# TritonDataCenter/containerpilot

Measured on AMD Instinct MI355X. Metric: events/sec, higher is better.
Workload: dtype n/a (CPU daemon, no tensor math; see BASELINE.json north_star); 1 GPU; model=containerpilot daemon, BASELINE stress shape scaled to 550 jobs, jobs=550, watches=50, parallelism=1 independent daemons (1/rank)

## Files before the change

### cpp/include/cpilot/loop.hpp

```cpp
#pragma once

#include <sys/types.h>

#include <chrono>
#include <cstdint>
#include <deque>
#include <functional>
#include <map>
#include <memory>
#include <mutex>
#include <queue>
#include <vector>

namespace cpilot {

using Clock = std::chrono::steady_clock;
using TimePoint = Clock::time_point;
using Ns = std::chrono::nanoseconds;

std::function<void()> timedItem(const char* tag, std::function<void()> fn);
void dumpItemTags();

void resetThreadScheduling();

class Loop {
 public:
  using FdCallback = std::function<void(uint32_t epollEvents)>;
  using TimerCallback = std::function<void()>;
  using ChildCallback = std::function<void(int waitStatus)>;

  Loop();
  ~Loop();

  Loop(const Loop&) = delete;
  Loop& operator=(const Loop&) = delete;

  void watchFd(int fd, uint32_t events, FdCallback cb);
  void modifyFd(int fd, uint32_t events);
  void unwatchFd(int fd);

  uint64_t addTimeout(Ns delay, TimerCallback cb);
  uint64_t addInterval(Ns interval, TimerCallback cb, Ns initialDelay = Ns(-1));
  void cancelTimer(uint64_t id);

  void defer(std::function<void()> fn);

  void post(std::function<void()> fn);

  void watchChild(pid_t pid, ChildCallback cb);
  void reapChildren();
  void notifyChildExit(pid_t pid, int status);

  static void postIfLive(Loop* loop, uint64_t id, std::function<void()> fn);
  uint64_t id() const { return id_; }

  void run();
  void stop();

  bool stopped() const { return stopped_; }

 private:
  struct Timer {
    uint64_t id;
    TimePoint deadline;
    Ns interval;
    TimerCallback cb;
    bool canceled = false;
  };
  struct TimerCmp {
    bool operator()(const std::shared_ptr<Timer>& a,
                    const std::shared_ptr<Timer>& b) const {
      return a->deadline > b->deadline;
    }
  };

  void armTimerFd();
  void fireDueTimers();
  void drainDeferred();
  void drainPosted();

  uint64_t id_ = 0;
  int epfd_ = -1;
  int timerfd_ = -1;
  int wakeupFds_[2] = {-1, -1};
  bool stopped_ = false;

  std::map<int, FdCallback> fdCallbacks_;
  std::priority_queue<std::shared_ptr<Timer>,
                      std::vector<std::shared_ptr<Timer>>, TimerCmp>
      timers_;
  std::map<uint64_t, std::shared_ptr<Timer>> timersById_;
  uint64_t nextTimerId_ = 1;

  std::deque<std::function<void()>> deferred_;

  std::mutex postedMu_;
  std::deque<std::function<void()>> posted_;

  std::map<pid_t, ChildCallback> children_;
  std::map<pid_t, int> unclaimedExits_;
};

}
```

### cpp/include/cpilot/spawner.hpp

```cpp
#pragma once

#include <sys/types.h>

#include <cstdint>
#include <deque>
#include <functional>
#include <map>
#include <memory>
#include <mutex>
#include <string>
#include <thread>
#include <vector>

#include "cpilot/loop.hpp"

namespace cpilot {

class Spawner {
 public:
  using SpawnCb = std::function<void(pid_t pid, int err)>;

  static Spawner& global();

  void spawn(Loop& loop, const std::string& execPath,
             const std::vector<std::string>& args,
             std::shared_ptr<const std::vector<std::string>> baseEnv,
             const std::vector<std::string>& extraEnv, int stdioFd,
             SpawnCb cb);

  int helperCount() const { return (int)helpers_.size(); }

  size_t backlog();
  bool overloaded();

 private:
  Spawner();
  struct Helper {
    int sock = -1;
    pid_t pid = -1;
    bool dead = false;
    std::deque<std::pair<std::vector<char>, int>> overflow;
    std::mutex sendMu;
  };
  struct Pending {
    Loop* loop;
    uint64_t loopId;
    SpawnCb cb;
    size_t helperIdx;
  };

  bool launchHelper(Helper* h);
  void flushOverflow(size_t idx);
  void readerMain();
  void handleMessage(size_t idx, const char* buf, size_t len);
  void helperDied(size_t idx);
  bool sendRequest(Helper& h, const std::vector<char>& buf, int fd);
  void wakeReader();

  std::string helperPath_;
  std::vector<std::unique_ptr<Helper>> helpers_;
  size_t nextHelper_ = 0;

  std::mutex mu_;
  std::map<uint32_t, Pending> pending_;
  uint32_t nextReqId_ = 1;
  std::map<pid_t, std::pair<Loop*, uint64_t>> pidLoops_;

  int wakeFds_[2] = {-1, -1};
  std::thread reader_;
};

}
```

### cpp/include/cpilot/spawnproto.hpp

```cpp
#pragma once

#include <cstdint>

namespace cpilot {
namespace spawnproto {

constexpr int kHelperFd = 3;

enum MsgType : uint32_t {
  kSpawnRequest = 1,
  kSpawnReply = 2,
  kChildExit = 3,
};

struct RequestHeader {
  uint32_t type;
  uint32_t reqId;
  uint32_t argc;
  uint32_t envc;
  uint8_t wantStdio;
  uint8_t pad[3];
};

struct Reply {
  uint32_t type;
  uint32_t reqId;
  int32_t pid;
  int32_t err;
};

struct ExitNotice {
  uint32_t type;
  uint32_t pad;
  int32_t pid;
  int32_t status;
};

constexpr size_t kMaxRequestBytes = 1024 * 1024;

}
}
```

### cpp/src/command.cpp

```cpp
#include "cpilot/command.hpp"

#include <fcntl.h>
#include <signal.h>
#include <sys/epoll.h>
#include <sys/wait.h>
#include <unistd.h>

#include <cctype>
#include <cstring>
#include <cstdio>
#include <map>

#include "cpilot/log.hpp"
#include "cpilot/spawner.hpp"

extern char** environ;

namespace cpilot {

namespace {

std::map<std::string, std::string>& pidEnvOverlay() {
  static std::map<std::string, std::string> overlay;
  return overlay;
}

std::shared_ptr<const std::vector<std::string>>& baseEnvCache() {
  static std::shared_ptr<const std::vector<std::string>> cache;
  return cache;
}
bool& baseEnvDirty() {
  static bool dirty = true;
  return dirty;
}

std::shared_ptr<const std::vector<std::string>> baseEnvSnapshot() {
  if (!baseEnvDirty() && baseEnvCache()) return baseEnvCache();
  auto& overlay = pidEnvOverlay();
  auto env = std::make_shared<std::vector<std::string>>();
  for (char** e = ::environ; *e; e++) {
    const char* eq = strchr(*e, '=');
    if (eq && overlay.count(std::string(*e, eq - *e))) continue;
    env->emplace_back(*e);
  }
  baseEnvCache() = env;
  baseEnvDirty() = false;
  return baseEnvCache();
}

std::vector<std::string>& overlayStrings() {
  static std::vector<std::string> strings;
  return strings;
}
std::map<std::string, size_t>& overlayIndex() {
  static std::map<std::string, size_t> index;
  return index;
}

const std::vector<std::string>& overlayExtras() { return overlayStrings(); }

void overlaySet(const std::string& key, const std::string& value) {
  auto [it, inserted] = pidEnvOverlay().emplace(key, value);
  if (inserted) {
    overlayIndex()[key] = overlayStrings().size();
    overlayStrings().push_back(key + "=" + value);
    if (getenv(key.c_str())) baseEnvDirty() = true;
  } else {
    it->second = value;
    overlayStrings()[overlayIndex()[key]] = key + "=" + value;
  }
}

void overlayErase(const std::string& key) {
  if (pidEnvOverlay().erase(key)) {
    auto idxIt = overlayIndex().find(key);
    if (idxIt != overlayIndex().end()) {
      size_t slot = idxIt->second;
      overlayIndex().erase(idxIt);
      auto& strs = overlayStrings();
      if (slot + 1 != strs.size()) {
        strs[slot] = std::move(strs.back());
        size_t eq = strs[slot].find('=');
        overlayIndex()[strs[slot].substr(0, eq)] = slot;
      }
      strs.pop_back();
    }
    if (getenv(key.c_str())) baseEnvDirty() = true;
  }
}

}

void commandEnvInvalidate() { baseEnvDirty() = true; }

bool parseArgs(const Json& raw, std::string* execPath,
               std::vector<std::string>* args, std::string* err) {
  std::vector<std::string> all;
  if (raw.isString()) {
    std::string s = raw.str();
    size_t a = 0, b = s.size();
    while (a < b && isspace((unsigned char)s[a])) a++;
    while (b > a && isspace((unsigned char)s[b - 1])) b--;
    s = s.substr(a, b - a);
    if (!s.empty()) {
      std::string cur;
      for (char c : s) {
        if (c == ' ') {
          all.push_back(cur);
          cur.clear();
        } else {
          cur += c;
        }
      }
      all.push_back(cur);
    }
  } else if (raw.isArray()) {
    for (auto& e : raw.array()) {
      if (e.isString()) all.push_back(e.str());
      else all.push_back(e.dump());
    }
  } else if (!raw.isNull()) {
    *err = "unable to parse exec arguments";
    return false;
  }
  if (all.empty()) {
    *err = "received zero-length argument";
    return false;
  }
  *execPath = all[0];
  args->assign(all.begin() + 1, all.end());
  return true;
}

CommandPtr newCommand(const Json& rawExec, Duration timeout, bool raw,
                      const std::string& logField, std::string* err) {
  std::string execPath;
  std::vector<std::string> args;
  if (!parseArgs(rawExec, &execPath, &args, err)) return nullptr;
  return std::make_shared<Command>(execPath, args, timeout, raw, logField);
}

Command::Command(std::string execPath, std::vector<std::string> args,
                 Duration timeout, bool raw, std::string logField)
    : name_(execPath),
      exec_(std::move(execPath)),
      args_(std::move(args)),
      timeout_(timeout),
      raw_(raw),
      logField_(std::move(logField)) {}

std::string Command::envName() const {
  if (name_.empty()) return name_;
  std::string name = name_;
  size_t slash = name.find_last_of('/');
  if (slash != std::string::npos) name = name.substr(slash + 1);
  size_t dot = name.find_last_of('.');
  if (dot != std::string::npos && dot > 0)
    name = name.substr(0, dot) + name.substr(name.size());
  std::string out;
  for (char c : name) {
    if (isalnum((unsigned char)c)) {
      out += (char)toupper((unsigned char)c);
    } else if (out.empty() || out.back() != '_') {
      out += '_';
    }
  }
  return out;
}

void Command::run(Loop& loop, std::shared_ptr<Bus> bus) {
  if (running_) {
    LOG_DEBUG("%s already running, queueing run", name_.c_str());
    pendingRun_ = true;
    return;
  }
  spawn(loop, std::move(bus));
}

void Command::spawn(Loop& loop, std::shared_ptr<Bus> bus) {
  loop_ = &loop;
  LOG_DEBUG("%s.Run start", name_.c_str());

  int pipefds[2] = {-1, -1};
  if (!raw_) {
    if (pipe2(pipefds, O_CLOEXEC) != 0) {
      LOG_ERROR("unable to create pipe for %s: %s", name_.c_str(),
                strerror(errno));
      bus->publish(Event{EventCode::ExitFailed, name_});
      bus->publish(Event{EventCode::Error, strerror(errno)});
      return;
    }
  }

  running_ = true;
  pid_ = -1;
  pendingSignal_ = 0;
  tReq_ = Clock::now();
  auto self = shared_from_this();
  int readFd = pipefds[0];
  auto baseEnv = baseEnvSnapshot();
  Spawner::SpawnCb compCb =
      [this, self, bus, readFd](pid_t pid, int err) {
        if (pid < 0) {
          LOG_ERROR("unable to start %s: %s", name_.c_str(), strerror(err));
          if (readFd >= 0) close(readFd);
          running_ = false;
          pendingRun_ = false;
          pendingSignal_ = 0;
          bus->publish(Event{EventCode::ExitFailed, name_});
          bus->publish(Event{EventCode::Error, strerror(err)});
          return;
        }
        pid_ = pid;
        tCb_ = Clock::now();
        if (pidEnvName_.empty())
          pidEnvName_ = "CONTAINERPILOT_" + envName() + "_PID";
        overlaySet(pidEnvName_, std::to_string(pid));

        if (!raw_) {
          logFd_ = readFd;
          fcntl(logFd_, F_SETFL, O_NONBLOCK);
          loop_->watchFd(logFd_, EPOLLIN | EPOLLHUP, [this, self](uint32_t) {
            char buf[4096];
            while (true) {
              ssize_t n = read(logFd_, buf, sizeof(buf));
              if (n > 0) {
                logBuf_.append(buf, n);
                size_t pos;
                while ((pos = logBuf_.find('\n')) != std::string::npos) {
                  logging::logFields(logging::Level::Info, logField_, pid_,
                                     logBuf_.substr(0, pos));
                  logBuf_.erase(0, pos + 1);
                }
              } else if (n == 0 || (n < 0 && errno != EAGAIN)) {
                if (!logBuf_.empty()) {
                  logging::logFields(logging::Level::Info, logField_, pid_,
                                     logBuf_);
                  logBuf_.clear();
                }
                loop_->unwatchFd(logFd_);
                close(logFd_);
                logFd_ = -1;
                return;
              } else {
                return;
              }
            }
          });
        }

        if (timeout_ > Duration(0)) {
          timeoutTimer_ = loop_->addTimeout(timeout_, [this, self] {
            LOG_WARN("%s timeout after %llds", name_.c_str(),
                     (long long)std::chrono::duration_cast<
                         std::chrono::seconds>(timeout_)
                         .count());
            timeoutTimer_ = 0;
            kill();
          });
        }

        if (pendingSignal_ != 0) {
          ::kill(-pid, pendingSignal_);
          pendingSignal_ = 0;
        }

        loop_->watchChild(pid, [this, self, bus](int status) {
          onExit(*loop_, bus, status);
        });
      };
  Spawner::global().spawn(loop, exec_, args_, std::move(baseEnv),
                          overlayExtras(), raw_ ? -1 : pipefds[1],
                          std::move(compCb));
}

void Command::onExit(Loop& loop, std::shared_ptr<Bus> bus, int status) {
  LOG_DEBUG("%s.Run end", name_.c_str());
  static const bool rttDebug = cpilotDebugEnv("CPILOT_LOOP_DEBUG");
  if (rttDebug) {
    auto now = Clock::now();
    double total =
        std::chrono::duration<double, std::milli>(now - tReq_).count();
    if (total > 50.0) {
      double execPhase =
          std::chrono::duration<double, std::milli>(now - tCb_).count();
      fprintf(stderr,
              "spawn rtt: %s total=%.0fms spawn_phase=%.0fms "
              "exec_phase=%.0fms\n",
              name_.c_str(), total, total - execPhase, execPhase);
    }
  }
  if (timeoutTimer_) {
    loop.cancelTimer(timeoutTimer_);
    timeoutTimer_ = 0;
  }
  if (logFd_ >= 0) {
    char buf[4096];
    ssize_t n;
    while ((n = read(logFd_, buf, sizeof(buf))) > 0) logBuf_.append(buf, n);
    size_t pos;
    while ((pos = logBuf_.find('\n')) != std::string::npos) {
      logging::logFields(logging::Level::Info, logField_, pid_,
                         logBuf_.substr(0, pos));
      logBuf_.erase(0, pos + 1);
    }
    if (!logBuf_.empty()) {
      logging::logFields(logging::Level::Info, logField_, pid_, logBuf_);
      logBuf_.clear();
    }
    loop.unwatchFd(logFd_);
    close(logFd_);
    logFd_ = -1;
  }

  if (!pidEnvName_.empty()) overlayErase(pidEnvName_);

  running_ = false;
  pid_ = -1;

  bool success = WIFEXITED(status) && WEXITSTATUS(status) == 0;
  if (success) {
    LOG_DEBUG("%s exited without error", name_.c_str());
    bus->publish(Event{EventCode::ExitSuccess, name_});
  } else {
    int code = WIFEXITED(status) ? WEXITSTATUS(status)
                                 : 128 + (WIFSIGNALED(status) ? WTERMSIG(status) : 0);
    LOG_ERROR("%s exited with error: exit status %d", name_.c_str(), code);
    bus->publish(Event{EventCode::ExitFailed, name_});
    bus->publish(Event{EventCode::Error,
                      name_ + ": exit status " + std::to_string(code)});
  }

  if (pendingRun_) {
    pendingRun_ = false;
    spawn(loop, bus);
  }
}

void Command::term() {
  LOG_DEBUG("%s.term", name_.c_str());
  if (pid_ > 0) {
    LOG_DEBUG("terminating command '%s' at pid: %d", name_.c_str(), pid_);
    ::kill(-pid_, SIGTERM);
  } else if (running_ && pendingSignal_ != SIGKILL) {
    pendingSignal_ = SIGTERM;
  }
}

void Command::kill() {
  LOG_DEBUG("%s.kill", name_.c_str());
  if (pid_ > 0) {
    LOG_DEBUG("killing command '%s' at pid: %d", name_.c_str(), pid_);
    ::kill(-pid_, SIGKILL);
  } else if (running_) {
    pendingSignal_ = SIGKILL;
  }
}

}
```

### cpp/src/loop.cpp

```cpp
#include "cpilot/loop.hpp"

#include <fcntl.h>
#include <sched.h>
#include <sys/resource.h>
#include <sys/epoll.h>
#include <sys/timerfd.h>
#include <sys/wait.h>
#include <unistd.h>

#include <cstdio>
#include <cstring>
#include <algorithm>
#include <set>
#include <stdexcept>

#include "cpilot/log.hpp"

namespace cpilot {

void resetThreadScheduling() {
  struct sched_param sp;
  memset(&sp, 0, sizeof(sp));
  sched_setscheduler(0, SCHED_OTHER, &sp);
  setpriority(PRIO_PROCESS, 0, 0);
}

namespace {
std::mutex& liveLoopsMu() {
  static std::mutex mu;
  return mu;
}
std::map<Loop*, uint64_t>& liveLoops() {
  static std::map<Loop*, uint64_t> loops;
  return loops;
}
uint64_t nextLoopId() {
  static uint64_t next = 1;
  return next++;
}
}

namespace {
struct ItemTagStats {
  double ms = 0;
  uint64_t count = 0;
};
std::map<std::string, ItemTagStats>& itemTags() {
  static std::map<std::string, ItemTagStats> tags;
  return tags;
}
}

std::function<void()> timedItem(const char* tag, std::function<void()> fn) {
  static const bool on = cpilotDebugEnv("CPILOT_LOOP_DEBUG");
  if (!on) return fn;
  std::string t(tag);
  return [t, fn = std::move(fn)] {
    TimePoint t0 = Clock::now();
    fn();
    auto& slot = itemTags()[t];
    slot.ms +=
        std::chrono::duration<double, std::milli>(Clock::now() - t0).count();
    slot.count++;
  };
}

void dumpItemTags() {
  for (auto& kv : itemTags())
    fprintf(stderr, "  item tag %s: %.0fms over %llu (avg %.1fus)\n",
            kv.first.c_str(), kv.second.ms,
            (unsigned long long)kv.second.count,
            kv.second.count ? kv.second.ms * 1000 / kv.second.count : 0.0);
  itemTags().clear();
}

void Loop::postIfLive(Loop* loop, uint64_t id, std::function<void()> fn) {
  std::lock_guard<std::mutex> l(liveLoopsMu());
  auto it = liveLoops().find(loop);
  if (it != liveLoops().end() && it->second == id) loop->post(std::move(fn));
}

Loop::Loop() {
  {
    std::lock_guard<std::mutex> l(liveLoopsMu());
    id_ = nextLoopId();
    liveLoops()[this] = id_;
  }
  epfd_ = epoll_create1(EPOLL_CLOEXEC);
  if (epfd_ < 0) throw std::runtime_error("epoll_create1 failed");
  timerfd_ = timerfd_create(CLOCK_MONOTONIC, TFD_NONBLOCK | TFD_CLOEXEC);
  if (timerfd_ < 0) throw std::runtime_error("timerfd_create failed");
  if (pipe2(wakeupFds_, O_NONBLOCK | O_CLOEXEC) != 0)
    throw std::runtime_error("pipe2 failed");

  watchFd(timerfd_, EPOLLIN, [this](uint32_t) {
    uint64_t expirations;
    while (read(timerfd_, &expirations, sizeof(expirations)) > 0) {
    }
    fireDueTimers();
  });
  watchFd(wakeupFds_[0], EPOLLIN, [this](uint32_t) {
    char buf[256];
    while (read(wakeupFds_[0], buf, sizeof(buf)) > 0) {
    }
    drainPosted();
  });
}

Loop::~Loop() {
  {
    std::lock_guard<std::mutex> l(liveLoopsMu());
    liveLoops().erase(this);
  }
  if (epfd_ >= 0) close(epfd_);
  if (timerfd_ >= 0) close(timerfd_);
  if (wakeupFds_[0] >= 0) close(wakeupFds_[0]);
  if (wakeupFds_[1] >= 0) close(wakeupFds_[1]);
}

void Loop::watchFd(int fd, uint32_t events, FdCallback cb) {
  struct epoll_event ev;
  memset(&ev, 0, sizeof(ev));
  ev.events = events;
  ev.data.fd = fd;
  if (epoll_ctl(epfd_, EPOLL_CTL_ADD, fd, &ev) != 0)
    throw std::runtime_error(std::string("epoll_ctl ADD failed: ") +
                             strerror(errno));
  fdCallbacks_[fd] = std::move(cb);
}

void Loop::modifyFd(int fd, uint32_t events) {
  struct epoll_event ev;
  memset(&ev, 0, sizeof(ev));
  ev.events = events;
  ev.data.fd = fd;
  epoll_ctl(epfd_, EPOLL_CTL_MOD, fd, &ev);
}

void Loop::unwatchFd(int fd) {
  epoll_ctl(epfd_, EPOLL_CTL_DEL, fd, nullptr);
  fdCallbacks_.erase(fd);
}

uint64_t Loop::addTimeout(Ns delay, TimerCallback cb) {
  auto t = std::make_shared<Timer>();
  t->id = nextTimerId_++;
  t->deadline = Clock::now() + delay;
  t->interval = Ns(0);
  t->cb = std::move(cb);
  timersById_[t->id] = t;
  timers_.push(t);
  armTimerFd();
  return t->id;
}

uint64_t Loop::addInterval(Ns interval, TimerCallback cb, Ns initialDelay) {
  if (interval <= Ns(0)) interval = Ns(1);
  if (initialDelay < Ns(0)) initialDelay = interval;
  auto t = std::make_shared<Timer>();
  t->id = nextTimerId_++;
  t->deadline = Clock::now() + initialDelay;
  t->interval = interval;
  t->cb = std::move(cb);
  timersById_[t->id] = t;
  timers_.push(t);
  armTimerFd();
  return t->id;
}

void Loop::cancelTimer(uint64_t id) {
  auto it = timersById_.find(id);
  if (it == timersById_.end()) return;
  it->second->canceled = true;
  timersById_.erase(it);
}

void Loop::defer(std::function<void()> fn) { deferred_.push_back(std::move(fn)); }

void Loop::post(std::function<void()> fn) {
  {
    std::lock_guard<std::mutex> l(postedMu_);
    posted_.push_back(std::move(fn));
  }
  char b = 1;
  ssize_t unused = write(wakeupFds_[1], &b, 1);
  (void)unused;
}

void Loop::watchChild(pid_t pid, ChildCallback cb) {
  auto it = unclaimedExits_.find(pid);
  if (it != unclaimedExits_.end()) {
    int status = it->second;
    unclaimedExits_.erase(it);
    cb(status);
    return;
  }
  children_[pid] = std::move(cb);
}

void Loop::reapChildren() {
  constexpr int kReapBatch = 64;
  int n = 0;
  while (n < kReapBatch) {
    int status = 0;
    pid_t pid = waitpid(-1, &status, WNOHANG);
    if (pid <= 0) return;
    n++;
    notifyChildExit(pid, status);
  }
  defer([this] { reapChildren(); });
}

void Loop::notifyChildExit(pid_t pid, int status) {
  auto it = children_.find(pid);
  if (it != children_.end()) {
    ChildCallback cb = std::move(it->second);
    children_.erase(it);
    cb(status);
  } else {
    unclaimedExits_[pid] = status;
  }
}

void Loop::armTimerFd() {
  while (!timers_.empty() && timers_.top()->canceled) timers_.pop();
  struct itimerspec its;
  memset(&its, 0, sizeof(its));
  if (!timers_.empty()) {
    auto now = Clock::now();
    Ns delta = std::chrono::duration_cast<Ns>(timers_.top()->deadline - now);
    if (delta < Ns(1)) delta = Ns(1);
    its.it_value.tv_sec = delta.count() / 1000000000LL;
    its.it_value.tv_nsec = delta.count() % 1000000000LL;
  }
  timerfd_settime(timerfd_, 0, &its, nullptr);
}

void Loop::fireDueTimers() {
  static const bool stallDebug = cpilotDebugEnv("CPILOT_LOOP_DEBUG");
  auto timeCb = [](Timer* t, const TimerCallback& cb) {
    if (!stallDebug) { cb(); return; }
    TimePoint t0 = Clock::now();
    cb();
    auto ms = std::chrono::duration<double, std::milli>(Clock::now() - t0)
                  .count();
    if (ms > 10.0)
      fprintf(stderr, "timer stall: id=%llu interval_ms=%lld took %.1f ms\n",
              (unsigned long long)t->id,
              (long long)(t->interval.count() / 1000000), ms);
  };
  auto now = Clock::now();
  while (!timers_.empty()) {
    auto t = timers_.top();
    if (t->canceled) {
      timers_.pop();
      continue;
    }
    if (t->deadline > now) break;
    timers_.pop();
    if (t->interval > Ns(0)) {
      t->deadline += t->interval;
      if (t->deadline <= now) {
        auto behind = std::chrono::duration_cast<Ns>(now - t->deadline);
        auto periods = behind.count() / t->interval.count() + 1;
        t->deadline += Ns(periods * t->interval.count());
      }
      timers_.push(t);
      timeCb(t.get(), t->cb);
    } else {
      auto keep = t;
      timersById_.erase(t->id);
      timeCb(keep.get(), keep->cb);
    }
  }
  armTimerFd();
}

void Loop::drainDeferred() {
  size_t n = deferred_.size();
  for (size_t i = 0; i < n && !deferred_.empty(); i++) {
    auto fn = std::move(deferred_.front());
    deferred_.pop_front();
    fn();
  }
}

void Loop::drainPosted() {
  constexpr auto kBudget = std::chrono::milliseconds(2);
  constexpr size_t kHardCap = 4096;
  TimePoint start = Clock::now();
  size_t processed = 0;
  bool more = true;
  while (more && processed < kHardCap &&
         Clock::now() - start < kBudget) {
    std::deque<std::function<void()>> batch;
    {
      std::lock_guard<std::mutex> l(postedMu_);
      for (size_t i = 0; i < 64 && !posted_.empty(); i++) {
        batch.push_back(std::move(posted_.front()));
        posted_.pop_front();
      }
      more = !posted_.empty();
    }
    static const bool itemDebug = cpilotDebugEnv("CPILOT_LOOP_DEBUG");
    if (itemDebug) {
      static double accMs = 0;
      static uint64_t nItems = 0, nSlow = 0;
      static TimePoint lastDump = Clock::now();
      for (auto& fn : batch) {
        TimePoint ti = Clock::now();
        fn();
        double ms = std::chrono::duration<double, std::milli>(
                        Clock::now() - ti).count();
        accMs += ms;
        nItems++;
        if (ms > 0.2) nSlow++;
      }
      if (Clock::now() - lastDump > std::chrono::seconds(5)) {
        fprintf(stderr,
                "posted items: %llu in 5s, total=%.0fms avg=%.1fus "
                "slow(>200us)=%llu\n",
                (unsigned long long)nItems, accMs,
                nItems ? accMs * 1000.0 / nItems : 0.0,
                (unsigned long long)nSlow);
        accMs = 0;
        nItems = nSlow = 0;
        lastDump = Clock::now();
      }
    } else {
      for (auto& fn : batch) fn();
    }
    processed += batch.size();
    if (batch.empty()) break;
  }
  if (more) {
    char b = 1;
    ssize_t unused = write(wakeupFds_[1], &b, 1);
    (void)unused;
  }
}

void Loop::run() {
  stopped_ = false;
  const bool stallDebug = cpilotDebugEnv("CPILOT_LOOP_DEBUG");
  auto probe = [stallDebug](const char* phase, TimePoint t0, int fd = -1) {
    if (!stallDebug) return;
    auto ms = std::chrono::duration<double, std::milli>(Clock::now() - t0)
                  .count();
    if (ms > 10.0)
      fprintf(stderr, "loop stall: %s fd=%d took %.1f ms\n", phase, fd, ms);
  };
  std::vector<struct epoll_event> events(64);
  double accDeferred = 0, accEpoll = 0, accFds = 0, accTimers = 0;
  std::map<int, std::pair<double, uint64_t>> accPerFd;
  uint64_t iters = 0;
  TimePoint lastReport = Clock::now();
  auto acc = [](double* slot, TimePoint t0) {
    *slot += std::chrono::duration<double, std::milli>(Clock::now() - t0)
                 .count();
  };
  while (!stopped_) {
    TimePoint t0 = Clock::now();
    drainDeferred();
    probe("drainDeferred", t0);
    if (stallDebug) acc(&accDeferred, t0);
    if (stopped_) break;
    armTimerFd();
    int timeoutMs = deferred_.empty() ? 1000 : 0;
    TimePoint te = Clock::now();
    int n = epoll_wait(epfd_, events.data(), (int)events.size(), timeoutMs);
    if (stallDebug) acc(&accEpoll, te);
    if (n < 0) {
      if (errno == EINTR) continue;
      LOG_ERROR("epoll_wait: %s", strerror(errno));
      break;
    }
    TimePoint tf = Clock::now();
    for (int i = 0; i < n && !stopped_; i++) {
      int fd = events[i].data.fd;
      auto it = fdCallbacks_.find(fd);
      if (it != fdCallbacks_.end()) {
        FdCallback cb = it->second;
        TimePoint tc = Clock::now();
        cb(events[i].events);
        probe("fdCallback", tc, fd);
        if (stallDebug) {
          auto& slot = accPerFd[fd];
          slot.first += std::chrono::duration<double, std::milli>(
                            Clock::now() - tc).count();
          slot.second++;
        }
      }
    }
    if (stallDebug) acc(&accFds, tf);
    TimePoint tt = Clock::now();
    fireDueTimers();
    probe("fireDueTimers", tt);
    if (stallDebug) {
      acc(&accTimers, tt);
      iters++;
      if (Clock::now() - lastReport > std::chrono::seconds(5)) {
        double secs = std::chrono::duration<double>(Clock::now() -
                                                    lastReport).count();
        fprintf(stderr,
                "loop phases: %.0f it/s deferred=%.0fms epoll=%.0fms "
                "fds=%.0fms timers=%.0fms (per %.1fs)\n",
                iters / secs, accDeferred, accEpoll, accFds, accTimers,
                secs);
        std::vector<std::pair<double, std::pair<int, uint64_t>>> top;
        for (auto& kv : accPerFd)
          top.push_back({kv.second.first, {kv.first, kv.second.second}});
        std::sort(top.rbegin(), top.rend());
        for (size_t k = 0; k < top.size() && k < 4; k++)
          fprintf(stderr, "  top fd %d: %.0fms over %llu events\n",
                  top[k].second.first, top[k].first,
                  (unsigned long long)top[k].second.second);
        dumpItemTags();
        accPerFd.clear();
        accDeferred = accEpoll = accFds = accTimers = 0;
        iters = 0;
        lastReport = Clock::now();
      }
    }
  }
}

void Loop::stop() { stopped_ = true; }

}
```

### cpp/src/spawner.cpp

```cpp
#include "cpilot/spawner.hpp"

#include <fcntl.h>
#include <limits.h>
#include <poll.h>
#include <signal.h>
#include <spawn.h>
#include <string.h>
#include <sys/socket.h>
#include <unistd.h>

#include <cstdio>
#include <cstdlib>

#include "cpilot/log.hpp"
#include "cpilot/spawnproto.hpp"

extern char** environ;

namespace cpilot {

using namespace spawnproto;

namespace {

int defaultHelperCount() {
  if (const char* v = getenv("CPILOT_SPAWN_HELPERS")) {
    int n = atoi(v);
    if (n >= 1 && n <= 64) return n;
  }
  long ncpu = sysconf(_SC_NPROCESSORS_ONLN);
  if (ncpu < 1) ncpu = 1;
  int n = (int)(ncpu / 16);
  if (n < 2) n = 2;
  if (n > 8) n = 8;
  return n;
}

std::string findHelperBinary() {
  if (const char* v = getenv("CPILOT_SPAWN_HELPER")) return v;
  char buf[PATH_MAX];
  ssize_t n = readlink("/proc/self/exe", buf, sizeof(buf) - 1);
  if (n > 0) {
    buf[n] = 0;
    std::string dir(buf);
    size_t slash = dir.find_last_of('/');
    if (slash != std::string::npos) {
      std::string candidate = dir.substr(0, slash) + "/cpilot-spawn-helper";
      if (access(candidate.c_str(), X_OK) == 0) return candidate;
    }
  }
  return "cpilot-spawn-helper";
}

bool spawnDebug() {
  static bool on = cpilotDebugEnv("CPILOT_SPAWN_DEBUG");
  return on;
}

}

Spawner& Spawner::global() {
  static Spawner* s = new Spawner();
  return *s;
}

Spawner::Spawner() {
  helperPath_ = findHelperBinary();
  if (pipe2(wakeFds_, O_NONBLOCK | O_CLOEXEC) != 0)
    LOG_ERROR("spawner: pipe2 failed: %s", strerror(errno));
  int n = defaultHelperCount();
  for (int i = 0; i < n; i++) helpers_.push_back(std::make_unique<Helper>());
  for (auto& h : helpers_) {
    if (!launchHelper(h.get())) {
      logging::logf(logging::Level::Fatal,
                    "spawner: cannot launch spawn helper '%s': %s",
                    helperPath_.c_str(), strerror(errno));
    }
  }
  reader_ = std::thread([this] { readerMain(); });
  reader_.detach();
}

bool Spawner::launchHelper(Helper* h) {
  int socks[2];
  if (socketpair(AF_UNIX, SOCK_SEQPACKET | SOCK_CLOEXEC, 0, socks) != 0)
    return false;
  int bufsz = 1 << 20;
  setsockopt(socks[0], SOL_SOCKET, SO_SNDBUF, &bufsz, sizeof(bufsz));
  setsockopt(socks[1], SOL_SOCKET, SO_SNDBUF, &bufsz, sizeof(bufsz));
  fcntl(socks[0], F_SETFL, O_NONBLOCK);

  posix_spawn_file_actions_t actions;
  posix_spawn_file_actions_init(&actions);
  posix_spawn_file_actions_adddup2(&actions, socks[1], kHelperFd);
  posix_spawnattr_t attr;
  posix_spawnattr_init(&attr);
  sigset_t empty;
  sigemptyset(&empty);
  posix_spawnattr_setsigmask(&attr, &empty);
  posix_spawnattr_setflags(&attr, POSIX_SPAWN_SETSIGMASK);

  char* argv[] = {const_cast<char*>("cpilot-spawn-helper"), nullptr};
  pid_t pid = -1;
  int rc = posix_spawn(&pid, helperPath_.c_str(), &actions, &attr, argv,
                       environ);
  posix_spawn_file_actions_destroy(&actions);
  posix_spawnattr_destroy(&attr);
  close(socks[1]);
  if (rc != 0) {
    close(socks[0]);
    errno = rc;
    return false;
  }
  h->sock = socks[0];
  h->pid = pid;
  h->dead = false;
  return true;
}

size_t Spawner::backlog() {
  std::lock_guard<std::mutex> l(mu_);
  return pending_.size();
}

void Spawner::flushOverflow(size_t idx) {
  Helper& h = *helpers_[idx];
  while (true) {
    std::deque<std::pair<std::vector<char>, int>> batch;
    {
      std::lock_guard<std::mutex> l(mu_);
      if (h.dead || h.overflow.empty()) return;
      for (int i = 0; i < 16 && !h.overflow.empty(); i++) {
        batch.push_back(std::move(h.overflow.front()));
        h.overflow.pop_front();
      }
    }
    size_t sent = 0;
    {
      std::lock_guard<std::mutex> sl(h.sendMu);
      for (auto& [buf, fd] : batch) {
        if (!sendRequest(h, buf, fd)) break;
        if (fd >= 0) close(fd);
        sent++;
      }
    }
    if (sent < batch.size()) {
      std::lock_guard<std::mutex> l(mu_);
      for (size_t i = batch.size(); i > sent; i--)
        h.overflow.push_front(std::move(batch[i - 1]));
      return;
    }
  }
}

bool Spawner::overloaded() {
  return backlog() > helpers_.size() * 16;
}

void Spawner::wakeReader() {
  char b = 1;
  ssize_t unused = write(wakeFds_[1], &b, 1);
  (void)unused;
}

void Spawner::spawn(Loop& loop, const std::string& execPath,
                    const std::vector<std::string>& args,
                    std::shared_ptr<const std::vector<std::string>> baseEnv,
                    const std::vector<std::string>& extraEnv, int stdioFd,
                    SpawnCb cb) {
  RequestHeader hdr;
  memset(&hdr, 0, sizeof(hdr));
  hdr.type = kSpawnRequest;
  hdr.argc = 1 + (uint32_t)args.size();
  hdr.envc = (uint32_t)((baseEnv ? baseEnv->size() : 0) + extraEnv.size());
  hdr.wantStdio = stdioFd >= 0 ? 1 : 0;

  size_t size = sizeof(hdr) + execPath.size() + 1;
  for (auto& a : args) size += a.size() + 1;
  if (baseEnv)
    for (auto& e : *baseEnv) size += e.size() + 1;
  for (auto& e : extraEnv) size += e.size() + 1;
  if (size > kMaxRequestBytes) {
    if (stdioFd >= 0) close(stdioFd);
    loop.post([cb] { cb(-1, E2BIG); });
    return;
  }

  std::vector<char> buf;
  buf.reserve(size);
  auto append = [&buf](const std::string& s) {
    buf.insert(buf.end(), s.begin(), s.end());
    buf.push_back('\0');
  };
  buf.resize(sizeof(hdr));
  append(execPath);
  for (auto& a : args) append(a);
  if (baseEnv)
    for (auto& e : *baseEnv) append(e);
  for (auto& e : extraEnv) append(e);

  size_t idx = 0;
  uint32_t reqId = 0;
  bool queued = false;
  {
    std::lock_guard<std::mutex> l(mu_);
    reqId = nextReqId_++;
    hdr.reqId = reqId;
    memcpy(buf.data(), &hdr, sizeof(hdr));

    bool found = false;
    for (size_t i = 0; i < helpers_.size(); i++) {
      idx = (nextHelper_ + i) % helpers_.size();
      if (!helpers_[idx]->dead) {
        found = true;
        break;
      }
    }
    nextHelper_ = (idx + 1) % helpers_.size();
    if (!found) {
      if (stdioFd >= 0) close(stdioFd);
      loop.post([cb] { cb(-1, ECHILD); });
      return;
    }
    pending_[reqId] = Pending{&loop, loop.id(), std::move(cb), idx};
    if (!helpers_[idx]->overflow.empty()) {
      helpers_[idx]->overflow.emplace_back(std::move(buf), stdioFd);
      queued = true;
    }
  }
  if (spawnDebug())
    fprintf(stderr, "[spawner] req %u -> helper %zu\n", reqId, idx);
  if (queued) {
    wakeReader();
    return;
  }
  Helper& h = *helpers_[idx];
  bool sent;
  {
    std::lock_guard<std::mutex> sl(h.sendMu);
    sent = sendRequest(h, buf, stdioFd);
  }
  if (!sent) {
    std::lock_guard<std::mutex> l(mu_);
    h.overflow.emplace_back(std::move(buf), stdioFd);
    wakeReader();
    return;
  }
  if (stdioFd >= 0) close(stdioFd);
}

bool Spawner::sendRequest(Helper& h, const std::vector<char>& buf, int fd) {
  struct iovec iov{const_cast<char*>(buf.data()), buf.size()};
  struct msghdr msg;
  memset(&msg, 0, sizeof(msg));
  msg.msg_iov = &iov;
  msg.msg_iovlen = 1;
  char cmsgBuf[CMSG_SPACE(sizeof(int))];
  if (fd >= 0) {
    memset(cmsgBuf, 0, sizeof(cmsgBuf));
    msg.msg_control = cmsgBuf;
    msg.msg_controllen = sizeof(cmsgBuf);
    struct cmsghdr* c = CMSG_FIRSTHDR(&msg);
    c->cmsg_level = SOL_SOCKET;
    c->cmsg_type = SCM_RIGHTS;
    c->cmsg_len = CMSG_LEN(sizeof(int));
    memcpy(CMSG_DATA(c), &fd, sizeof(int));
  }
  while (true) {
    ssize_t n = sendmsg(h.sock, &msg, MSG_NOSIGNAL);
    if (spawnDebug())
      fprintf(stderr, "[spawner] sendmsg fd=%d n=%zd errno=%d\n", h.sock, n,
              n < 0 ? errno : 0);
    if (n >= 0) return true;
    if (errno == EINTR) continue;
    return false;
  }
}

void Spawner::readerMain() {
  resetThreadScheduling();
  std::vector<char> buf(64);
  while (true) {
    std::vector<struct pollfd> fds;
    {
      std::lock_guard<std::mutex> l(mu_);
      for (auto& h : helpers_) {
        short ev = h->dead ? 0 : POLLIN;
        if (!h->dead && !h->overflow.empty()) ev |= POLLOUT;
        fds.push_back({h->sock, ev, 0});
      }
    }
    fds.push_back({wakeFds_[0], POLLIN, 0});
    int rc = poll(fds.data(), (nfds_t)fds.size(), 1000);
    if (spawnDebug() && rc != 0) {
      fprintf(stderr, "[spawner] poll rc=%d", rc);
      for (size_t i = 0; i < fds.size(); i++)
        fprintf(stderr, " fd%d=%x", fds[i].fd, fds[i].revents);
      fprintf(stderr, "\n");
    }
    if (rc < 0) {
      if (errno == EINTR) continue;
      return;
    }
    if (fds.back().revents & POLLIN) {
      char drain[256];
      while (read(wakeFds_[0], drain, sizeof(drain)) > 0) {
      }
    }
    for (size_t i = 0; i + 1 < fds.size(); i++) {
      if (fds[i].revents & POLLOUT) flushOverflow(i);
      if (fds[i].revents & (POLLIN | POLLHUP | POLLERR)) {
        while (true) {
          ssize_t n = recv(fds[i].fd, buf.data(), buf.size(), MSG_DONTWAIT);
          if (n > 0) {
            if (spawnDebug())
              fprintf(stderr, "[spawner] msg from helper %zu len=%zd\n", i, n);
            handleMessage(i, buf.data(), (size_t)n);
            continue;
          }
          if (n < 0 && (errno == EAGAIN || errno == EINTR)) break;
          if (spawnDebug())
            fprintf(stderr, "[spawner] helper %zu died n=%zd errno=%d\n",
                    i, n, errno);
          helperDied(i);
          break;
        }
      }
    }
  }
}

void Spawner::handleMessage(size_t idx, const char* data, size_t len) {
  uint32_t type = 0;
  if (len >= sizeof(uint32_t)) memcpy(&type, data, sizeof(type));
  if (spawnDebug() && type != kSpawnReply && type != kChildExit)
    fprintf(stderr, "[spawner] DROP unknown msg type=%u len=%zu\n", type, len);
  if (type == kSpawnReply && len >= sizeof(Reply)) {
    Reply r;
    memcpy(&r, data, sizeof(r));
    Pending p;
    {
      std::lock_guard<std::mutex> l(mu_);
      auto it = pending_.find(r.reqId);
      if (it == pending_.end()) {
        if (spawnDebug())
          fprintf(stderr, "[spawner] DROP reply for unknown req %u\n",
                  r.reqId);
        return;
      }
      p = std::move(it->second);
      pending_.erase(it);
    }
    if (spawnDebug())
      fprintf(stderr, "[spawner] reply req %u pid %d\n", r.reqId, r.pid);
    if (r.pid > 0) pidLoops_[r.pid] = {p.loop, p.loopId};
    SpawnCb cb = std::move(p.cb);
    pid_t pid = r.pid;
    int err = r.err;
    Loop::postIfLive(p.loop, p.loopId,
                     timedItem("spawncb", [cb, pid, err] { cb(pid, err); }));
  } else if (type == kChildExit && len >= sizeof(ExitNotice)) {
    ExitNotice note;
    memcpy(&note, data, sizeof(note));
    auto it = pidLoops_.find(note.pid);
    if (it == pidLoops_.end()) {
      if (spawnDebug())
        fprintf(stderr, "[spawner] DROP exit notice for unknown pid %d\n",
                note.pid);
      return;
    }
    if (spawnDebug())
      fprintf(stderr, "[spawner] exit pid %d\n", note.pid);
    auto [loop, loopId] = it->second;
    pidLoops_.erase(it);
    pid_t pid = note.pid;
    int status = note.status;
    Loop::postIfLive(loop, loopId, timedItem("exit", [loop, pid, status] {
                       loop->notifyChildExit(pid, status);
                     }));
  }
}

void Spawner::helperDied(size_t idx) {
  std::vector<Pending> lost;
  {
    std::lock_guard<std::mutex> l(mu_);
    Helper& h = *helpers_[idx];
    if (h.dead) return;
    h.dead = true;
    LOG_ERROR("spawner: helper %d (pid %d) died; respawning",
              (int)idx, (int)h.pid);
    for (auto it = pending_.begin(); it != pending_.end();) {
      if (it->second.helperIdx == idx) {
        lost.push_back(std::move(it->second));
        it = pending_.erase(it);
      } else {
        ++it;
      }
    }
    for (auto& [obuf, ofd] : h.overflow)
      if (ofd >= 0) close(ofd);
    h.overflow.clear();
    close(h.sock);
    if (!launchHelper(&h)) {
      LOG_ERROR("spawner: helper respawn failed: %s", strerror(errno));
      h.dead = true;
    }
  }
  for (auto& p : lost) {
    SpawnCb cb = std::move(p.cb);
    Loop::postIfLive(p.loop, p.loopId, [cb] { cb(-1, ECHILD); });
  }
}

}
```

### cpp/src/spawnhelper_main.cpp

```cpp
#include <errno.h>
#include <fcntl.h>
#include <poll.h>
#include <signal.h>
#include <sched.h>
#include <spawn.h>
#include <sys/resource.h>
#include <stdio.h>
#include <stdlib.h>
#include <string.h>
#include <sys/socket.h>
#include <sys/wait.h>
#include <unistd.h>

#include <vector>

#include "cpilot/spawnproto.hpp"

using namespace cpilot::spawnproto;

namespace {

int selfPipe[2] = {-1, -1};

bool helperDebug() {
  const char* v = getenv("CPILOT_SPAWN_DEBUG");
  static bool on = v && v[0] && !(v[0] == '0' && !v[1]);
  return on;
}

void onSigchld(int) {
  char b = 1;
  ssize_t unused = write(selfPipe[1], &b, 1);
  (void)unused;
}

bool sendAll(int fd, const void* buf, size_t len) {
  while (true) {
    ssize_t n = send(fd, buf, len, MSG_NOSIGNAL);
    if (n == (ssize_t)len) return true;
    if (n < 0 && (errno == EINTR)) continue;
    if (n < 0 && errno == EAGAIN) {
      struct pollfd p{fd, POLLOUT, 0};
      poll(&p, 1, 1000);
      continue;
    }
    return false;
  }
}

void reapAndNotify(int sock) {
  while (true) {
    int status = 0;
    pid_t pid = waitpid(-1, &status, WNOHANG);
    if (pid <= 0) return;
    if (helperDebug())
      fprintf(stderr, "[helper %d] reaped pid %d\n", getpid(), (int)pid);
    ExitNotice note{kChildExit, 0, (int32_t)pid, (int32_t)status};
    if (!sendAll(sock, &note, sizeof(note))) _exit(0);
  }
}

void handleRequest(int sock, const char* buf, size_t len, int stdioFd) {
  if (len < sizeof(RequestHeader)) return;
  RequestHeader hdr;
  memcpy(&hdr, buf, sizeof(hdr));
  const char* p = buf + sizeof(hdr);
  const char* end = buf + len;

  std::vector<const char*> argv, envp;
  for (uint32_t i = 0; i < hdr.argc + hdr.envc && p < end; i++) {
    if (i < hdr.argc)
      argv.push_back(p);
    else
      envp.push_back(p);
    p += strnlen(p, end - p) + 1;
  }
  Reply reply{kSpawnReply, hdr.reqId, -1, EINVAL};
  if (argv.size() == hdr.argc && envp.size() == hdr.envc && !argv.empty()) {
    argv.push_back(nullptr);
    envp.push_back(nullptr);

    posix_spawnattr_t attr;
    posix_spawnattr_init(&attr);
    sigset_t empty;
    sigemptyset(&empty);
    posix_spawnattr_setsigmask(&attr, &empty);
    posix_spawnattr_setpgroup(&attr, 0);
    short flags = POSIX_SPAWN_SETPGROUP | POSIX_SPAWN_SETSIGMASK;
#ifdef POSIX_SPAWN_USEVFORK
    flags |= POSIX_SPAWN_USEVFORK;
#endif
    posix_spawnattr_setflags(&attr, flags);

    posix_spawn_file_actions_t actions;
    posix_spawn_file_actions_init(&actions);
    if (hdr.wantStdio && stdioFd >= 0) {
      posix_spawn_file_actions_adddup2(&actions, stdioFd, 1);
      posix_spawn_file_actions_adddup2(&actions, stdioFd, 2);
    }
    pid_t pid = -1;
    int rc = posix_spawnp(&pid, argv[0], &actions, &attr,
                          const_cast<char**>(argv.data()),
                          const_cast<char**>(envp.data()));
    posix_spawn_file_actions_destroy(&actions);
    posix_spawnattr_destroy(&attr);
    reply.pid = (rc == 0) ? (int32_t)pid : -1;
    reply.err = rc;
    if (helperDebug())
      fprintf(stderr, "[helper %d] spawned pid %d req %u\n", getpid(),
              (int)pid, hdr.reqId);
  }
  if (stdioFd >= 0) close(stdioFd);
  if (!sendAll(sock, &reply, sizeof(reply))) _exit(0);
}

}

int cpilotSpawnHelperMain() {
  {
    struct sched_param sp;
    memset(&sp, 0, sizeof(sp));
    sched_setscheduler(0, SCHED_OTHER, &sp);
    setpriority(PRIO_PROCESS, 0, 0);
  }
  const int sock = kHelperFd;
  fcntl(sock, F_SETFD, FD_CLOEXEC);
  if (pipe2(selfPipe, O_NONBLOCK | O_CLOEXEC) != 0) _exit(1);

  struct sigaction sa;
  memset(&sa, 0, sizeof(sa));
  sa.sa_handler = onSigchld;
  sa.sa_flags = SA_RESTART | SA_NOCLDSTOP;
  sigaction(SIGCHLD, &sa, nullptr);
  signal(SIGPIPE, SIG_IGN);
  sigset_t none;
  sigemptyset(&none);
  sigprocmask(SIG_SETMASK, &none, nullptr);

  std::vector<char> buf(kMaxRequestBytes);
  char cmsgBuf[CMSG_SPACE(sizeof(int))];

  while (true) {
    struct pollfd fds[2] = {{sock, POLLIN, 0}, {selfPipe[0], POLLIN, 0}};
    int rc = poll(fds, 2, -1);
    if (helperDebug())
      fprintf(stderr, "[helper %d] poll rc=%d sock=%x pipe=%x\n", getpid(),
              rc, fds[0].revents, fds[1].revents);
    if (rc < 0) {
      if (errno == EINTR) {
        reapAndNotify(sock);
        continue;
      }
      _exit(1);
    }
    if (fds[1].revents & POLLIN) {
      char drain[256];
      while (read(selfPipe[0], drain, sizeof(drain)) > 0) {
      }
      reapAndNotify(sock);
    }
    if (fds[0].revents & (POLLIN | POLLHUP | POLLERR)) {
      struct iovec iov{buf.data(), buf.size()};
      struct msghdr msg;
      memset(&msg, 0, sizeof(msg));
      msg.msg_iov = &iov;
      msg.msg_iovlen = 1;
      msg.msg_control = cmsgBuf;
      msg.msg_controllen = sizeof(cmsgBuf);
      ssize_t n = recvmsg(sock, &msg, MSG_CMSG_CLOEXEC);
      if (helperDebug())
        fprintf(stderr, "[helper %d] recvmsg n=%zd errno=%d\n", getpid(), n,
                n < 0 ? errno : 0);
      if (n == 0) _exit(0);
      if (n < 0) {
        if (errno == EINTR || errno == EAGAIN) continue;
        _exit(0);
      }
      int passedFd = -1;
      for (struct cmsghdr* c = CMSG_FIRSTHDR(&msg); c;
           c = CMSG_NXTHDR(&msg, c)) {
        if (c->cmsg_level == SOL_SOCKET && c->cmsg_type == SCM_RIGHTS)
          memcpy(&passedFd, CMSG_DATA(c), sizeof(int));
      }
      handleRequest(sock, buf.data(), (size_t)n, passedFd);
      reapAndNotify(sock);
    }
  }
}

#ifndef CPILOT_HELPER_NO_MAIN
int main() { return cpilotSpawnHelperMain(); }
#endif
```

Measured before the change: 11000 events/s.

## Send environment deltas to spawn helpers and batch loop wakeups and posts

Spawn requests no longer carry the full environment. The spawner keeps a sequenced log of overlay changes and sends only deltas since the last state each helper acknowledged. Each helper keeps its own environment table and asks for a resync when its sequence does not match. Reader-thread replies are batched per loop through postMany, loop wakeup writes are coalesced with an atomic flag, and the timerfd is rearmed only when the earliest deadline changes. Together these cut per-spawn serialization, syscalls and lock traffic, at the cost of a more complex protocol with resync and generation tracking that could misbehave on desync.

```diff
diff --git a/cpp/include/cpilot/loop.hpp b/cpp/include/cpilot/loop.hpp
--- a/cpp/include/cpilot/loop.hpp
+++ b/cpp/include/cpilot/loop.hpp
@@ -2,6 +2,7 @@
 
 #include <sys/types.h>
 
+#include <atomic>
 #include <chrono>
 #include <cstdint>
 #include <deque>
@@ -46,13 +47,21 @@
   void defer(std::function<void()> fn);
 
   void post(std::function<void()> fn);
+  void postMany(std::vector<std::function<void()>>&& fns);
 
   void watchChild(pid_t pid, ChildCallback cb);
   void reapChildren();
   void notifyChildExit(pid_t pid, int status);
 
   static void postIfLive(Loop* loop, uint64_t id, std::function<void()> fn);
+  static void postManyIfLive(Loop* loop, uint64_t id,
+                             std::vector<std::function<void()>>&& fns);
   uint64_t id() const { return id_; }
+
+  uint64_t timerArmCalls() const { return timerArmCalls_; }
+  uint64_t wakeWrites() const {
+    return wakeWrites_.load(std::memory_order_relaxed);
+  }
 
   void run();
   void stop();
@@ -75,6 +84,7 @@
   };
 
   void armTimerFd();
+  void wake();
   void fireDueTimers();
   void drainDeferred();
   void drainPosted();
@@ -91,11 +101,16 @@
       timers_;
   std::map<uint64_t, std::shared_ptr<Timer>> timersById_;
   uint64_t nextTimerId_ = 1;
+  bool timerArmed_ = false;
+  TimePoint armedDeadline_{};
+  uint64_t timerArmCalls_ = 0;
 
   std::deque<std::function<void()>> deferred_;
 
   std::mutex postedMu_;
   std::deque<std::function<void()>> posted_;
+  std::atomic<bool> wakePending_{false};
+  std::atomic<uint64_t> wakeWrites_{0};
 
   std::map<pid_t, ChildCallback> children_;
   std::map<pid_t, int> unclaimedExits_;
diff --git a/cpp/include/cpilot/spawner.hpp b/cpp/include/cpilot/spawner.hpp
--- a/cpp/include/cpilot/spawner.hpp
+++ b/cpp/include/cpilot/spawner.hpp
@@ -2,6 +2,7 @@
 
 #include <sys/types.h>
 
+#include <atomic>
 #include <cstdint>
 #include <deque>
 #include <functional>
@@ -10,6 +11,7 @@
 #include <mutex>
 #include <string>
 #include <thread>
+#include <unordered_map>
 #include <vector>
 
 #include "cpilot/loop.hpp"
@@ -22,49 +24,112 @@
 
   static Spawner& global();
 
+  void envSet(const std::string& name, const std::string& value);
+  void envErase(const std::string& name);
+  static void envInvalidate();
+
   void spawn(Loop& loop, const std::string& execPath,
-             const std::vector<std::string>& args,
-             std::shared_ptr<const std::vector<std::string>> baseEnv,
-             const std::vector<std::string>& extraEnv, int stdioFd,
-             SpawnCb cb);
+             const std::vector<std::string>& args, int stdioFd, SpawnCb cb);
 
   int helperCount() const { return (int)helpers_.size(); }
 
   size_t backlog();
   bool overloaded();
 
+  struct Stats {
+    uint64_t fullSent = 0;
+    uint64_t deltaSent = 0;
+    uint64_t envBytes = 0;
+    uint64_t resyncs = 0;
+    uint64_t overflowQueued = 0;
+  };
+  Stats stats() const;
+  pid_t helperPid(size_t idx);
+  void desyncHelper(size_t idx);
+
  private:
   Spawner();
+  struct Queued {
+    std::vector<char> buf;
+    int fd;
+    uint64_t gen;
+  };
   struct Helper {
     int sock = -1;
     pid_t pid = -1;
-    bool dead = false;
-    std::deque<std::pair<std::vector<char>, int>> overflow;
+    std::atomic<bool> dead{false};
+    std::atomic<uint64_t> gen{0};
+    std::deque<Queued> overflow;
+    bool flushing = false;
     std::mutex sendMu;
+    uint64_t sentSeq = 0;
+    uint64_t sentEpoch = 0;
+    uint64_t sentGen = UINT64_MAX;
+    bool desyncOnce = false;
   };
   struct Pending {
     Loop* loop;
     uint64_t loopId;
     SpawnCb cb;
     size_t helperIdx;
+    uint64_t gen;
+    int stdioFd;
+    std::string argv;
+    uint32_t argc;
+    bool resent = false;
+  };
+  struct EnvOp {
+    uint64_t seq;
+    std::string name;
+    std::string kv;
+  };
+  struct PostItem {
+    Loop* loop;
+    uint64_t loopId;
+    std::function<void()> fn;
   };
 
-  bool launchHelper(Helper* h);
+  bool launchHelper(Helper* h,
+                    const std::shared_ptr<const std::vector<std::string>>& env);
   void flushOverflow(size_t idx);
   void readerMain();
   void handleMessage(size_t idx, const char* buf, size_t len);
   void helperDied(size_t idx);
   bool sendRequest(Helper& h, const std::vector<char>& buf, int fd);
+  void sendOrQueue(Helper& h, Queued&& q);
   void wakeReader();
+  void flushPosts();
+  void resend(uint32_t reqId);
+
+  void refreshBase();
+  void logOp(const std::string& name, std::string kv);
+  void trimLog();
+  bool appendEnv(Helper& h, uint64_t gen, bool forceFull,
+                 std::vector<char>* buf);
 
   std::string helperPath_;
+  int sndbuf_ = 1 << 20;
   std::vector<std::unique_ptr<Helper>> helpers_;
   size_t nextHelper_ = 0;
 
-  std::mutex mu_;
+  std::unordered_map<std::string, std::string> overlay_;
+  std::shared_ptr<const std::vector<std::string>> base_;
+  static bool baseDirty_;
+  uint64_t baseEpoch_ = 0;
+  size_t baseBytes_ = 0, overlayBytes_ = 0;
+  uint64_t envSeq_ = 0;
+  std::deque<EnvOp> envLog_;
+  std::vector<const EnvOp*> deltaOps_;
+
+  mutable std::mutex mu_;
   std::map<uint32_t, Pending> pending_;
   uint32_t nextReqId_ = 1;
+  std::shared_ptr<const std::vector<std::string>> launchEnv_;
   std::map<pid_t, std::pair<Loop*, uint64_t>> pidLoops_;
+  std::vector<PostItem> posts_;
+
+  std::atomic<uint64_t> nFull_{0}, nDelta_{0}, nEnvBytes_{0}, nResync_{0},
+      nOverflow_{0};
 
   int wakeFds_[2] = {-1, -1};
   std::thread reader_;
diff --git a/cpp/include/cpilot/spawnproto.hpp b/cpp/include/cpilot/spawnproto.hpp
--- a/cpp/include/cpilot/spawnproto.hpp
+++ b/cpp/include/cpilot/spawnproto.hpp
@@ -1,5 +1,6 @@
 #pragma once
 
+#include <cstddef>
 #include <cstdint>
 
 namespace cpilot {
@@ -11,15 +12,20 @@
   kSpawnRequest = 1,
   kSpawnReply = 2,
   kChildExit = 3,
+  kSpawnResync = 4,
 };
 
 struct RequestHeader {
   uint32_t type;
   uint32_t reqId;
   uint32_t argc;
-  uint32_t envc;
+  uint32_t envSetc;
+  uint32_t envUnsetc;
   uint8_t wantStdio;
-  uint8_t pad[3];
+  uint8_t envFull;
+  uint8_t pad[2];
+  uint64_t envFrom;
+  uint64_t envTo;
 };
 
 struct Reply {
diff --git a/cpp/src/command.cpp b/cpp/src/command.cpp
--- a/cpp/src/command.cpp
+++ b/cpp/src/command.cpp
@@ -14,84 +14,21 @@
 #include "cpilot/log.hpp"
 #include "cpilot/spawner.hpp"
 
-extern char** environ;
-
 namespace cpilot {
 
 namespace {
 
-std::map<std::string, std::string>& pidEnvOverlay() {
-  static std::map<std::string, std::string> overlay;
-  return overlay;
-}
-
-std::shared_ptr<const std::vector<std::string>>& baseEnvCache() {
-  static std::shared_ptr<const std::vector<std::string>> cache;
-  return cache;
-}
-bool& baseEnvDirty() {
-  static bool dirty = true;
-  return dirty;
-}
-
-std::shared_ptr<const std::vector<std::string>> baseEnvSnapshot() {
-  if (!baseEnvDirty() && baseEnvCache()) return baseEnvCache();
-  auto& overlay = pidEnvOverlay();
-  auto env = std::make_shared<std::vector<std::string>>();
-  for (char** e = ::environ; *e; e++) {
-    const char* eq = strchr(*e, '=');
-    if (eq && overlay.count(std::string(*e, eq - *e))) continue;
-    env->emplace_back(*e);
-  }
-  baseEnvCache() = env;
-  baseEnvDirty() = false;
-  return baseEnvCache();
-}
-
-std::vector<std::string>& overlayStrings() {
-  static std::vector<std::string> strings;
-  return strings;
-}
-std::map<std::string, size_t>& overlayIndex() {
-  static std::map<std::string, size_t> index;
-  return index;
-}
-
-const std::vector<std::string>& overlayExtras() { return overlayStrings(); }
-
 void overlaySet(const std::string& key, const std::string& value) {
-  auto [it, inserted] = pidEnvOverlay().emplace(key, value);
-  if (inserted) {
-    overlayIndex()[key] = overlayStrings().size();
-    overlayStrings().push_back(key + "=" + value);
-    if (getenv(key.c_str())) baseEnvDirty() = true;
-  } else {
-    it->second = value;
-    overlayStrings()[overlayIndex()[key]] = key + "=" + value;
-  }
+  Spawner::global().envSet(key, value);
 }
 
 void overlayErase(const std::string& key) {
-  if (pidEnvOverlay().erase(key)) {
-    auto idxIt = overlayIndex().find(key);
-    if (idxIt != overlayIndex().end()) {
-      size_t slot = idxIt->second;
-      overlayIndex().erase(idxIt);
-      auto& strs = overlayStrings();
-      if (slot + 1 != strs.size()) {
-        strs[slot] = std::move(strs.back());
-        size_t eq = strs[slot].find('=');
-        overlayIndex()[strs[slot].substr(0, eq)] = slot;
-      }
-      strs.pop_back();
-    }
-    if (getenv(key.c_str())) baseEnvDirty() = true;
-  }
-}
-
-}
-
-void commandEnvInvalidate() { baseEnvDirty() = true; }
+  Spawner::global().envErase(key);
+}
+
+}
+
+void commandEnvInvalidate() { Spawner::envInvalidate(); }
 
 bool parseArgs(const Json& raw, std::string* execPath,
                std::vector<std::string>* args, std::string* err) {
@@ -198,7 +135,6 @@
   tReq_ = Clock::now();
   auto self = shared_from_this();
   int readFd = pipefds[0];
-  auto baseEnv = baseEnvSnapshot();
   Spawner::SpawnCb compCb =
       [this, self, bus, readFd](pid_t pid, int err) {
         if (pid < 0) {
@@ -269,8 +205,7 @@
           onExit(*loop_, bus, status);
         });
       };
-  Spawner::global().spawn(loop, exec_, args_, std::move(baseEnv),
-                          overlayExtras(), raw_ ? -1 : pipefds[1],
+  Spawner::global().spawn(loop, exec_, args_, raw_ ? -1 : pipefds[1],
                           std::move(compCb));
 }
 
diff --git a/cpp/src/loop.cpp b/cpp/src/loop.cpp
--- a/cpp/src/loop.cpp
+++ b/cpp/src/loop.cpp
@@ -80,6 +80,14 @@
   if (it != liveLoops().end() && it->second == id) loop->post(std::move(fn));
 }
 
+void Loop::postManyIfLive(Loop* loop, uint64_t id,
+                          std::vector<std::function<void()>>&& fns) {
+  std::lock_guard<std::mutex> l(liveLoopsMu());
+  auto it = liveLoops().find(loop);
+  if (it != liveLoops().end() && it->second == id)
+    loop->postMany(std::move(fns));
+}
+
 Loop::Loop() {
   {
     std::lock_guard<std::mutex> l(liveLoopsMu());
@@ -97,6 +105,7 @@
     uint64_t expirations;
     while (read(timerfd_, &expirations, sizeof(expirations)) > 0) {
     }
+    timerArmed_ = false;
     fireDueTimers();
   });
   watchFd(wakeupFds_[0], EPOLLIN, [this](uint32_t) {
@@ -182,6 +191,22 @@
     std::lock_guard<std::mutex> l(postedMu_);
     posted_.push_back(std::move(fn));
   }
+  wake();
+}
+
+void Loop::postMany(std::vector<std::function<void()>>&& fns) {
+  if (fns.empty()) return;
+  {
+    std::lock_guard<std::mutex> l(postedMu_);
+    for (auto& fn : fns) posted_.push_back(std::move(fn));
+  }
+  fns.clear();
+  wake();
+}
+
+void Loop::wake() {
+  if (wakePending_.exchange(true)) return;
+  wakeWrites_.fetch_add(1, std::memory_order_relaxed);
   char b = 1;
   ssize_t unused = write(wakeupFds_[1], &b, 1);
   (void)unused;
@@ -226,13 +251,21 @@
   while (!timers_.empty() && timers_.top()->canceled) timers_.pop();
   struct itimerspec its;
   memset(&its, 0, sizeof(its));
-  if (!timers_.empty()) {
+  if (timers_.empty()) {
+    if (!timerArmed_) return;
+    timerArmed_ = false;
+  } else {
+    TimePoint deadline = timers_.top()->deadline;
+    if (timerArmed_ && deadline == armedDeadline_) return;
     auto now = Clock::now();
-    Ns delta = std::chrono::duration_cast<Ns>(timers_.top()->deadline - now);
+    Ns delta = std::chrono::duration_cast<Ns>(deadline - now);
     if (delta < Ns(1)) delta = Ns(1);
     its.it_value.tv_sec = delta.count() / 1000000000LL;
     its.it_value.tv_nsec = delta.count() % 1000000000LL;
-  }
+    timerArmed_ = true;
+    armedDeadline_ = deadline;
+  }
+  timerArmCalls_++;
   timerfd_settime(timerfd_, 0, &its, nullptr);
 }
 
@@ -291,6 +324,7 @@
   TimePoint start = Clock::now();
   size_t processed = 0;
   bool more = true;
+  wakePending_.store(false);
   while (more && processed < kHardCap &&
          Clock::now() - start < kBudget) {
     std::deque<std::function<void()>> batch;
@@ -333,11 +367,7 @@
     processed += batch.size();
     if (batch.empty()) break;
   }
-  if (more) {
-    char b = 1;
-    ssize_t unused = write(wakeupFds_[1], &b, 1);
-    (void)unused;
-  }
+  if (more) wake();
 }
 
 void Loop::run() {
diff --git a/cpp/src/spawner.cpp b/cpp/src/spawner.cpp
--- a/cpp/src/spawner.cpp
+++ b/cpp/src/spawner.cpp
@@ -9,8 +9,11 @@
 #include <sys/socket.h>
 #include <unistd.h>
 
+#include <cstddef>
 #include <cstdio>
 #include <cstdlib>
+#include <string_view>
+#include <unordered_set>
 
 #include "cpilot/log.hpp"
 #include "cpilot/spawnproto.hpp"
@@ -68,10 +71,14 @@
   helperPath_ = findHelperBinary();
   if (pipe2(wakeFds_, O_NONBLOCK | O_CLOEXEC) != 0)
     LOG_ERROR("spawner: pipe2 failed: %s", strerror(errno));
+  if (const char* v = getenv("CPILOT_SPAWN_SNDBUF")) {
+    int b = atoi(v);
+    if (b > 0) sndbuf_ = b;
+  }
   int n = defaultHelperCount();
   for (int i = 0; i < n; i++) helpers_.push_back(std::make_unique<Helper>());
   for (auto& h : helpers_) {
-    if (!launchHelper(h.get())) {
+    if (!launchHelper(h.get(), nullptr)) {
       logging::logf(logging::Level::Fatal,
                     "spawner: cannot launch spawn helper '%s': %s",
                     helperPath_.c_str(), strerror(errno));
@@ -81,11 +88,12 @@
   reader_.detach();
 }
 
-bool Spawner::launchHelper(Helper* h) {
+bool Spawner::launchHelper(
+    Helper* h, const std::shared_ptr<const std::vector<std::string>>& env) {
   int socks[2];
   if (socketpair(AF_UNIX, SOCK_SEQPACKET | SOCK_CLOEXEC, 0, socks) != 0)
     return false;
-  int bufsz = 1 << 20;
+  int bufsz = sndbuf_;
   setsockopt(socks[0], SOL_SOCKET, SO_SNDBUF, &bufsz, sizeof(bufsz));
   setsockopt(socks[1], SOL_SOCKET, SO_SNDBUF, &bufsz, sizeof(bufsz));
   fcntl(socks[0], F_SETFL, O_NONBLOCK);
@@ -100,10 +108,15 @@
   posix_spawnattr_setsigmask(&attr, &empty);
   posix_spawnattr_setflags(&attr, POSIX_SPAWN_SETSIGMASK);
 
+  std::vector<char*> envp;
+  if (env) {
+    for (auto& e : *env) envp.push_back(const_cast<char*>(e.c_str()));
+    envp.push_back(nullptr);
+  }
   char* argv[] = {const_cast<char*>("cpilot-spawn-helper"), nullptr};
   pid_t pid = -1;
   int rc = posix_spawn(&pid, helperPath_.c_str(), &actions, &attr, argv,
-                       environ);
+                       env ? envp.data() : environ);
   posix_spawn_file_actions_destroy(&actions);
   posix_spawnattr_destroy(&attr);
   close(socks[1]);
@@ -123,10 +136,172 @@
   return pending_.size();
 }
 
+Spawner::Stats Spawner::stats() const {
+  Stats s;
+  s.fullSent = nFull_;
+  s.deltaSent = nDelta_;
+  s.envBytes = nEnvBytes_;
+  s.resyncs = nResync_;
+  s.overflowQueued = nOverflow_;
+  return s;
+}
+
+pid_t Spawner::helperPid(size_t idx) {
+  std::lock_guard<std::mutex> l(mu_);
+  return idx < helpers_.size() ? helpers_[idx]->pid : -1;
+}
+
+void Spawner::desyncHelper(size_t idx) {
+  if (idx < helpers_.size()) helpers_[idx]->desyncOnce = true;
+}
+
+
+void Spawner::logOp(const std::string& name, std::string kv) {
+  envLog_.push_back(EnvOp{++envSeq_, name, std::move(kv)});
+  if (envLog_.size() > 65536) envLog_.pop_front();
+}
+
+void Spawner::envSet(const std::string& name, const std::string& value) {
+  std::string kv = name + "=" + value;
+  auto [it, inserted] = overlay_.emplace(name, kv);
+  if (inserted) {
+    if (getenv(name.c_str())) baseDirty_ = true;
+  } else {
+    if (it->second == kv) return;
+    overlayBytes_ -= it->second.size() + 1;
+    it->second = kv;
+  }
+  overlayBytes_ += kv.size() + 1;
+  logOp(name, std::move(kv));
+}
+
+void Spawner::envErase(const std::string& name) {
+  auto it = overlay_.find(name);
+  if (it == overlay_.end()) return;
+  overlayBytes_ -= it->second.size() + 1;
+  overlay_.erase(it);
+  if (getenv(name.c_str())) baseDirty_ = true;
+  logOp(name, std::string());
+}
+
+bool Spawner::baseDirty_ = true;
+
+void Spawner::envInvalidate() { baseDirty_ = true; }
+
+void Spawner::refreshBase() {
+  if (!baseDirty_ && base_) return;
+  auto env = std::make_shared<std::vector<std::string>>();
+  size_t bytes = 0;
+  for (char** e = ::environ; *e; e++) {
+    const char* eq = strchr(*e, '=');
+    if (eq && overlay_.count(std::string(*e, eq - *e))) continue;
+    env->emplace_back(*e);
+    bytes += env->back().size() + 1;
+  }
+  base_ = env;
+  baseBytes_ = bytes;
+  baseDirty_ = false;
+  baseEpoch_++;
+  envSeq_++;
+  envLog_.clear();
+  std::lock_guard<std::mutex> l(mu_);
+  launchEnv_ = base_;
+}
+
+void Spawner::trimLog() {
+  uint64_t oldest = envSeq_;
+  for (auto& h : helpers_)
+    if (!h->dead && h->sentGen == h->gen && h->sentEpoch == baseEpoch_ &&
+        h->sentSeq < oldest)
+      oldest = h->sentSeq;
+  while (!envLog_.empty() && envLog_.front().seq <= oldest)
+    envLog_.pop_front();
+}
+
+bool Spawner::appendEnv(Helper& h, uint64_t gen, bool forceFull,
+                        std::vector<char>* buf) {
+  RequestHeader hdr;
+  memcpy(&hdr, buf->data(), sizeof(hdr));
+  auto append = [buf](const std::string& s) {
+    buf->insert(buf->end(), s.begin(), s.end());
+    buf->push_back('\0');
+  };
+  const size_t fullBytes = baseBytes_ + overlayBytes_;
+  bool full = forceFull || h.sentGen != gen || h.sentEpoch != baseEpoch_ ||
+              h.sentSeq > envSeq_;
+  if (!full && h.sentSeq != envSeq_) {
+    if (envLog_.empty() || envLog_.front().seq > h.sentSeq + 1) full = true;
+  }
+  deltaOps_.clear();
+  size_t deltaBytes = 0;
+  if (!full) {
+    std::unordered_set<std::string_view> seen;
+    for (auto it = envLog_.rbegin();
+         it != envLog_.rend() && it->seq > h.sentSeq; ++it) {
+      bool dup = false;
+      if (deltaOps_.size() < 16) {
+        for (const EnvOp* op : deltaOps_)
+          if (op->name == it->name) {
+            dup = true;
+            break;
+          }
+      } else {
+        if (seen.empty())
+          for (const EnvOp* op : deltaOps_) seen.insert(op->name);
+        dup = !seen.insert(it->name).second;
+      }
+      if (dup) continue;
+      deltaOps_.push_back(&*it);
+      deltaBytes += (it->kv.empty() ? it->name.size() : it->kv.size()) + 1;
+      if (deltaBytes > fullBytes) {
+        full = true;
+        break;
+      }
+    }
+  }
+  size_t envBytes = full ? fullBytes : deltaBytes;
+  if (buf->size() + envBytes > kMaxRequestBytes) return false;
+  buf->reserve(buf->size() + envBytes);
+  if (full) {
+    hdr.envFull = 1;
+    hdr.envSetc = (uint32_t)(base_->size() + overlay_.size());
+    hdr.envUnsetc = 0;
+    for (auto& e : *base_) append(e);
+    for (auto& kv : overlay_) append(kv.second);
+    nFull_++;
+  } else {
+    hdr.envFull = 0;
+    hdr.envSetc = hdr.envUnsetc = 0;
+    for (const EnvOp* op : deltaOps_)
+      if (!op->kv.empty()) {
+        append(op->kv);
+        hdr.envSetc++;
+      }
+    for (const EnvOp* op : deltaOps_)
+      if (op->kv.empty()) {
+        append(op->name);
+        hdr.envUnsetc++;
+      }
+    nDelta_++;
+  }
+  nEnvBytes_ += envBytes;
+  hdr.envFrom = h.sentSeq;
+  if (!full && h.desyncOnce) {
+    hdr.envFrom += 1000;
+    h.desyncOnce = false;
+  }
+  hdr.envTo = envSeq_;
+  memcpy(buf->data(), &hdr, sizeof(hdr));
+  h.sentSeq = envSeq_;
+  h.sentEpoch = baseEpoch_;
+  h.sentGen = gen;
+  return true;
+}
+
 void Spawner::flushOverflow(size_t idx) {
   Helper& h = *helpers_[idx];
   while (true) {
-    std::deque<std::pair<std::vector<char>, int>> batch;
+    std::deque<Queued> batch;
     {
       std::lock_guard<std::mutex> l(mu_);
       if (h.dead || h.overflow.empty()) return;
@@ -134,18 +309,19 @@
         batch.push_back(std::move(h.overflow.front()));
         h.overflow.pop_front();
       }
+      h.flushing = true;
     }
     size_t sent = 0;
     {
       std::lock_guard<std::mutex> sl(h.sendMu);
-      for (auto& [buf, fd] : batch) {
-        if (!sendRequest(h, buf, fd)) break;
-        if (fd >= 0) close(fd);
+      for (auto& q : batch) {
+        if (q.gen == h.gen && !sendRequest(h, q.buf, q.fd)) break;
         sent++;
       }
     }
+    std::lock_guard<std::mutex> l(mu_);
+    h.flushing = false;
     if (sent < batch.size()) {
-      std::lock_guard<std::mutex> l(mu_);
       for (size_t i = batch.size(); i > sent; i--)
         h.overflow.push_front(std::move(batch[i - 1]));
       return;
@@ -164,67 +340,77 @@
 }
 
 void Spawner::spawn(Loop& loop, const std::string& execPath,
-                    const std::vector<std::string>& args,
-                    std::shared_ptr<const std::vector<std::string>> baseEnv,
-                    const std::vector<std::string>& extraEnv, int stdioFd,
+                    const std::vector<std::string>& args, int stdioFd,
                     SpawnCb cb) {
+  refreshBase();
+
   RequestHeader hdr;
   memset(&hdr, 0, sizeof(hdr));
   hdr.type = kSpawnRequest;
   hdr.argc = 1 + (uint32_t)args.size();
-  hdr.envc = (uint32_t)((baseEnv ? baseEnv->size() : 0) + extraEnv.size());
   hdr.wantStdio = stdioFd >= 0 ? 1 : 0;
 
-  size_t size = sizeof(hdr) + execPath.size() + 1;
-  for (auto& a : args) size += a.size() + 1;
-  if (baseEnv)
-    for (auto& e : *baseEnv) size += e.size() + 1;
-  for (auto& e : extraEnv) size += e.size() + 1;
-  if (size > kMaxRequestBytes) {
+  size_t argvBytes = execPath.size() + 1;
+  for (auto& a : args) argvBytes += a.size() + 1;
+  if (sizeof(hdr) + argvBytes > kMaxRequestBytes) {
     if (stdioFd >= 0) close(stdioFd);
     loop.post([cb] { cb(-1, E2BIG); });
     return;
   }
-
-  std::vector<char> buf;
-  buf.reserve(size);
-  auto append = [&buf](const std::string& s) {
-    buf.insert(buf.end(), s.begin(), s.end());
-    buf.push_back('\0');
+  Queued q;
+  q.fd = stdioFd;
+  q.buf.reserve(sizeof(hdr) + argvBytes + 256);
+  q.buf.resize(sizeof(hdr));
+  auto append = [&q](const std::string& s) {
+    q.buf.insert(q.buf.end(), s.begin(), s.end());
+    q.buf.push_back('\0');
   };
-  buf.resize(sizeof(hdr));
   append(execPath);
   for (auto& a : args) append(a);
-  if (baseEnv)
-    for (auto& e : *baseEnv) append(e);
-  for (auto& e : extraEnv) append(e);
 
   size_t idx = 0;
+  bool found = false;
+  for (size_t i = 0; i < helpers_.size(); i++) {
+    idx = (nextHelper_ + i) % helpers_.size();
+    if (!helpers_[idx]->dead) {
+      found = true;
+      break;
+    }
+  }
+  nextHelper_ = (idx + 1) % helpers_.size();
+  if (!found) {
+    if (stdioFd >= 0) close(stdioFd);
+    loop.post([cb] { cb(-1, ECHILD); });
+    return;
+  }
+  Helper& h = *helpers_[idx];
+  q.gen = h.gen;
+  memcpy(q.buf.data(), &hdr, sizeof(hdr));
+  if (!appendEnv(h, q.gen, false, &q.buf)) {
+    if (stdioFd >= 0) close(stdioFd);
+    loop.post([cb] { cb(-1, E2BIG); });
+    return;
+  }
+  trimLog();
+
   uint32_t reqId = 0;
   bool queued = false;
   {
     std::lock_guard<std::mutex> l(mu_);
-    reqId = nextReqId_++;
-    hdr.reqId = reqId;
-    memcpy(buf.data(), &hdr, sizeof(hdr));
-
-    bool found = false;
-    for (size_t i = 0; i < helpers_.size(); i++) {
-      idx = (nextHelper_ + i) % helpers_.size();
-      if (!helpers_[idx]->dead) {
-        found = true;
-        break;
-      }
-    }
-    nextHelper_ = (idx + 1) % helpers_.size();
-    if (!found) {
+    if (h.dead || h.gen != q.gen) {
       if (stdioFd >= 0) close(stdioFd);
       loop.post([cb] { cb(-1, ECHILD); });
       return;
     }
-    pending_[reqId] = Pending{&loop, loop.id(), std::move(cb), idx};
-    if (!helpers_[idx]->overflow.empty()) {
-      helpers_[idx]->overflow.emplace_back(std::move(buf), stdioFd);
+    reqId = nextReqId_++;
+    memcpy(q.buf.data() + offsetof(RequestHeader, reqId), &reqId,
+           sizeof(reqId));
+    Pending p{&loop, loop.id(), std::move(cb), idx, q.gen, stdioFd,
+              std::string(q.buf.data() + sizeof(hdr), argvBytes), hdr.argc};
+    pending_.emplace(reqId, std::move(p));
+    if (!h.overflow.empty() || h.flushing) {
+      h.overflow.push_back(std::move(q));
+      nOverflow_++;
       queued = true;
     }
   }
@@ -234,19 +420,72 @@
     wakeReader();
     return;
   }
-  Helper& h = *helpers_[idx];
+  sendOrQueue(h, std::move(q));
+}
+
+void Spawner::sendOrQueue(Helper& h, Queued&& q) {
   bool sent;
   {
     std::lock_guard<std::mutex> sl(h.sendMu);
-    sent = sendRequest(h, buf, stdioFd);
+    if (h.gen != q.gen) return;
+    sent = sendRequest(h, q.buf, q.fd);
   }
   if (!sent) {
     std::lock_guard<std::mutex> l(mu_);
-    h.overflow.emplace_back(std::move(buf), stdioFd);
+    if (h.gen != q.gen) return;
+    h.overflow.push_back(std::move(q));
+    nOverflow_++;
+    wakeReader();
+  }
+}
+
+void Spawner::resend(uint32_t reqId) {
+  refreshBase();
+  RequestHeader hdr;
+  memset(&hdr, 0, sizeof(hdr));
+  Queued q;
+  Helper* h = nullptr;
+  {
+    std::lock_guard<std::mutex> l(mu_);
+    auto it = pending_.find(reqId);
+    if (it == pending_.end()) return;
+    Pending& p = it->second;
+    h = helpers_[p.helperIdx].get();
+    hdr.type = kSpawnRequest;
+    hdr.reqId = reqId;
+    hdr.argc = p.argc;
+    hdr.wantStdio = p.stdioFd >= 0 ? 1 : 0;
+    q.fd = p.stdioFd;
+    q.gen = p.gen;
+    q.buf.resize(sizeof(hdr));
+    memcpy(q.buf.data(), &hdr, sizeof(hdr));
+    q.buf.insert(q.buf.end(), p.argv.begin(), p.argv.end());
+  }
+  bool ok = appendEnv(*h, q.gen, true, &q.buf);
+  bool queued = false;
+  {
+    std::lock_guard<std::mutex> l(mu_);
+    auto it = pending_.find(reqId);
+    if (it == pending_.end()) return;
+    if (!ok) {
+      Pending p = std::move(it->second);
+      pending_.erase(it);
+      if (p.stdioFd >= 0) close(p.stdioFd);
+      SpawnCb cb = std::move(p.cb);
+      Loop::postIfLive(p.loop, p.loopId, [cb] { cb(-1, E2BIG); });
+      return;
+    }
+    if (!h->overflow.empty() || h->flushing) {
+      h->overflow.push_back(std::move(q));
+      nOverflow_++;
+      queued = true;
+    }
+  }
+  if (queued) {
     wakeReader();
     return;
   }
-  if (stdioFd >= 0) close(stdioFd);
+  sendOrQueue(*h, std::move(q));
 }
 
 bool Spawner::sendRequest(Helper& h, const std::vector<char>& buf, int fd) {
@@ -277,6 +516,21 @@
   }
 }
 
+void Spawner::flushPosts() {
+  size_t i = 0;
+  while (i < posts_.size()) {
+    Loop* loop = posts_[i].loop;
+    uint64_t loopId = posts_[i].loopId;
+    std::vector<std::function<void()>> fns;
+    for (; i < posts_.size() && posts_[i].loop == loop &&
+           posts_[i].loopId == loopId;
+         i++)
+      fns.push_back(std::move(posts_[i].fn));
+    Loop::postManyIfLive(loop, loopId, std::move(fns));
+  }
+  posts_.clear();
+}
+
 void Spawner::readerMain() {
   resetThreadScheduling();
   std::vector<char> buf(64);
@@ -287,7 +541,7 @@
       for (auto& h : helpers_) {
         short ev = h->dead ? 0 : POLLIN;
         if (!h->dead && !h->overflow.empty()) ev |= POLLOUT;
-        fds.push_back({h->sock, ev, 0});
+        fds.push_back({h->dead ? -1 : h->sock, ev, 0});
       }
     }
     fds.push_back({wakeFds_[0], POLLIN, 0});
@@ -316,6 +570,7 @@
             if (spawnDebug())
               fprintf(stderr, "[spawner] msg from helper %zu len=%zd\n", i, n);
             handleMessage(i, buf.data(), (size_t)n);
+            if (posts_.size() >= 256) flushPosts();
             continue;
           }
           if (n < 0 && (errno == EAGAIN || errno == EINTR)) break;
@@ -327,15 +582,43 @@
         }
       }
     }
+    flushPosts();
   }
 }
 
 void Spawner::handleMessage(size_t idx, const char* data, size_t len) {
   uint32_t type = 0;
   if (len >= sizeof(uint32_t)) memcpy(&type, data, sizeof(type));
-  if (spawnDebug() && type != kSpawnReply && type != kChildExit)
+  if (spawnDebug() && type != kSpawnReply && type != kChildExit &&
+      type != kSpawnResync)
     fprintf(stderr, "[spawner] DROP unknown msg type=%u len=%zu\n", type, len);
-  if (type == kSpawnReply && len >= sizeof(Reply)) {
+  if (type == kSpawnResync && len >= sizeof(Reply)) {
+    Reply r;
+    memcpy(&r, data, sizeof(r));
+    nResync_++;
+    Pending failed;
+    bool fail = false;
+    {
+      std::lock_guard<std::mutex> l(mu_);
+      auto it = pending_.find(r.reqId);
+      if (it == pending_.end()) return;
+      Pending& p = it->second;
+      if (!p.resent) {
+        p.resent = true;
+        uint32_t reqId = r.reqId;
+        posts_.push_back({p.loop, p.loopId, [this, reqId] { resend(reqId); }});
+      } else {
+        failed = std::move(p);
+        pending_.erase(it);
+        fail = true;
+      }
+    }
+    if (fail) {
+      if (failed.stdioFd >= 0) close(failed.stdioFd);
+      SpawnCb cb = std::move(failed.cb);
+      posts_.push_back({failed.loop, failed.loopId, [cb] { cb(-1, EPROTO); }});
+    }
+  } else if (type == kSpawnReply && len >= sizeof(Reply)) {
     Reply r;
     memcpy(&r, data, sizeof(r));
     Pending p;
@@ -353,12 +636,13 @@
     }
     if (spawnDebug())
       fprintf(stderr, "[spawner] reply req %u pid %d\n", r.reqId, r.pid);
+    if (p.stdioFd >= 0) close(p.stdioFd);
     if (r.pid > 0) pidLoops_[r.pid] = {p.loop, p.loopId};
     SpawnCb cb = std::move(p.cb);
     pid_t pid = r.pid;
     int err = r.err;
-    Loop::postIfLive(p.loop, p.loopId,
-                     timedItem("spawncb", [cb, pid, err] { cb(pid, err); }));
+    posts_.push_back({p.loop, p.loopId,
+                      timedItem("spawncb", [cb, pid, err] { cb(pid, err); })});
   } else if (type == kChildExit && len >= sizeof(ExitNotice)) {
     ExitNotice note;
     memcpy(&note, data, sizeof(note));
@@ -375,9 +659,9 @@
     pidLoops_.erase(it);
     pid_t pid = note.pid;
     int status = note.status;
-    Loop::postIfLive(loop, loopId, timedItem("exit", [loop, pid, status] {
-                       loop->notifyChildExit(pid, status);
-                     }));
+    posts_.push_back({loop, loopId, timedItem("exit", [loop, pid, status] {
+                        loop->notifyChildExit(pid, status);
+                      })});
   }
 }
 
@@ -387,7 +671,9 @@
     std::lock_guard<std::mutex> l(mu_);
     Helper& h = *helpers_[idx];
     if (h.dead) return;
+    std::lock_guard<std::mutex> sl(h.sendMu);
     h.dead = true;
+    h.gen++;
     LOG_ERROR("spawner: helper %d (pid %d) died; respawning",
               (int)idx, (int)h.pid);
     for (auto it = pending_.begin(); it != pending_.end();) {
@@ -398,19 +684,19 @@
         ++it;
       }
     }
-    for (auto& [obuf, ofd] : h.overflow)
-      if (ofd >= 0) close(ofd);
     h.overflow.clear();
     close(h.sock);
-    if (!launchHelper(&h)) {
+    h.sock = -1;
+    if (!launchHelper(&h, launchEnv_)) {
       LOG_ERROR("spawner: helper respawn failed: %s", strerror(errno));
       h.dead = true;
     }
   }
   for (auto& p : lost) {
+    if (p.stdioFd >= 0) close(p.stdioFd);
     SpawnCb cb = std::move(p.cb);
-    Loop::postIfLive(p.loop, p.loopId, [cb] { cb(-1, ECHILD); });
-  }
-}
-
-}
+    posts_.push_back({p.loop, p.loopId, [cb] { cb(-1, ECHILD); }});
+  }
+}
+
+}
diff --git a/cpp/src/spawnhelper_main.cpp b/cpp/src/spawnhelper_main.cpp
--- a/cpp/src/spawnhelper_main.cpp
+++ b/cpp/src/spawnhelper_main.cpp
@@ -12,6 +12,8 @@
 #include <sys/wait.h>
 #include <unistd.h>
 
+#include <string>
+#include <unordered_map>
 #include <vector>
 
 #include "cpilot/spawnproto.hpp"
@@ -60,6 +62,50 @@
   }
 }
 
+struct EnvTable {
+  std::vector<char*> envp{nullptr};
+  std::unordered_map<std::string, size_t> slots;
+  uint64_t seq = 0;
+  bool valid = false;
+
+  static std::string nameOf(const char* kv) {
+    const char* eq = strchr(kv, '=');
+    return eq ? std::string(kv, eq - kv) : std::string(kv);
+  }
+  void clear() {
+    for (char* e : envp) free(e);
+    envp.assign(1, nullptr);
+    slots.clear();
+  }
+  void set(const char* kv) {
+    char* copy = strdup(kv);
+    if (!copy) _exit(1);
+    auto [it, inserted] = slots.emplace(nameOf(kv), envp.size() - 1);
+    if (inserted) {
+      envp.back() = copy;
+      envp.push_back(nullptr);
+    } else {
+      free(envp[it->second]);
+      envp[it->second] = copy;
+    }
+  }
+  void unset(const char* name) {
+    auto it = slots.find(name);
+    if (it == slots.end()) return;
+    size_t slot = it->second, last = envp.size() - 2;
+    slots.erase(it);
+    free(envp[slot]);
+    if (slot != last) {
+      envp[slot] = envp[last];
+      slots[nameOf(envp[slot])] = slot;
+    }
+    envp[last] = nullptr;
+    envp.pop_back();
+  }
+};
+
+EnvTable envTable;
+
 void handleRequest(int sock, const char* buf, size_t len, int stdioFd) {
   if (len < sizeof(RequestHeader)) return;
   RequestHeader hdr;
@@ -67,18 +113,38 @@
   const char* p = buf + sizeof(hdr);
   const char* end = buf + len;
 
-  std::vector<const char*> argv, envp;
-  for (uint32_t i = 0; i < hdr.argc + hdr.envc && p < end; i++) {
+  bool wellFormed = len > sizeof(hdr) && end[-1] == '\0';
+  std::vector<const char*> argv, sets, unsets;
+  uint64_t total = (uint64_t)hdr.argc + hdr.envSetc + hdr.envUnsetc;
+  for (uint64_t i = 0; wellFormed && i < total && p < end; i++) {
     if (i < hdr.argc)
       argv.push_back(p);
+    else if (i < (uint64_t)hdr.argc + hdr.envSetc)
+      sets.push_back(p);
     else
-      envp.push_back(p);
+      unsets.push_back(p);
     p += strnlen(p, end - p) + 1;
   }
   Reply reply{kSpawnReply, hdr.reqId, -1, EINVAL};
-  if (argv.size() == hdr.argc && envp.size() == hdr.envc && !argv.empty()) {
+  if (wellFormed && argv.size() == hdr.argc && sets.size() == hdr.envSetc &&
+      unsets.size() == hdr.envUnsetc && !argv.empty()) {
+    if (!hdr.envFull && (!envTable.valid || envTable.seq != hdr.envFrom)) {
+      if (helperDebug())
+        fprintf(stderr, "[helper %d] resync req %u: have %llu, delta from %llu\n",
+                getpid(), hdr.reqId, (unsigned long long)envTable.seq,
+                (unsigned long long)hdr.envFrom);
+      if (stdioFd >= 0) close(stdioFd);
+      reply.type = kSpawnResync;
+      reply.err = 0;
+      if (!sendAll(sock, &reply, sizeof(reply))) _exit(0);
+      return;
+    }
+    if (hdr.envFull) envTable.clear();
+    for (const char* kv : sets) envTable.set(kv);
+    for (const char* name : unsets) envTable.unset(name);
+    envTable.seq = hdr.envTo;
+    envTable.valid = true;
     argv.push_back(nullptr);
-    envp.push_back(nullptr);
 
     posix_spawnattr_t attr;
     posix_spawnattr_init(&attr);
@@ -101,7 +167,7 @@
     pid_t pid = -1;
     int rc = posix_spawnp(&pid, argv[0], &actions, &attr,
                           const_cast<char**>(argv.data()),
-                          const_cast<char**>(envp.data()));
+                          envTable.envp.data());
     posix_spawn_file_actions_destroy(&actions);
     posix_spawnattr_destroy(&attr);
     reply.pid = (rc == 0) ? (int32_t)pid : -1;
```

New measurement: 10990 events/s. No clear change (-0.1%).
